# CederGroupHub/chgnet

Hardware: NVIDIA H100
Metric: structures_per_sec_EFS (higher is better)
Workload: dtype f32

## Files before the change

### chgnet_b200/_lib.py

```python
from __future__ import annotations

import ctypes
import os
from ctypes import c_char_p, c_double, c_float, c_int32, c_int64, c_void_p

import torch
from torch import Tensor

_HERE = os.path.dirname(os.path.abspath(__file__))
LIB_PATH = os.path.join(_HERE, "libchgnet_b200.so")

P, I, F, D, I64 = c_void_p, c_int32, c_float, c_double, c_int64

SIGNATURES: dict[str, list] = {
    "chg_embed_atoms": [P, P, I, P, P],
    "chg_edge_geometry": [P, P, P, P, P, P, I, P, P, P, P],
    "chg_bond_basis_embed": [P, P, I, P, P, I, F, F, I, P, P, P, P, P, P],
    "chg_bond_basis_bwd": [P, P, I, P, P, I, F, F, I, P, P, P, P, P, P, P],
    "chg_angle_basis_embed": [P, P, P, I, P, I, P, P, P, P],
    "chg_angle_basis_bwd": [P, P, P, I, P, I, P, P, P, P, P],
    "chg_linear": [P, P, I, I, P, P, P, P, I, P, P],
    "chg_gather_rows": [P, P, I, I, P, P],
    "chg_scatter_rows": [P, P, I, I, P, P],
    "chg_atom_conv_fwd": [P, P, P, P, P, P, I, P, P, P, P, P, P, P],
    "chg_atom_conv_bwd": [P, P, P, P, P, P, I, P, P, P, P, P, P, P, P, P],
    "chg_segment_sum": [P, I, P, P, I, I, I, P, I, P],
    "chg_atom_conv_fused": [P, P, P, P, P, P, P, I, I, P, P, P, P, P, P, P],
    "chg_bond_conv_fused": [P, P, P, P, P, P, P, P, I, I, P, P, P, P, P, P, P, P],
    "chg_bond_conv_fwd": [P, P, P, P, P, P, P, I, P, P, P, P, P, P, P],
    "chg_bond_conv_bwd": [P, P, P, P, P, I, P, P, P, P, P, P, P, P, P],
    "chg_angle_update_fwd": [P, P, P, P, P, P, P, I, P, P, P, P],
    "chg_angle_update_bwd": [P, P, I, P, P, P, P],
    "chg_readout": [P, P, P, I, P, P, P, P, I, P, F, P, P, P, P, P, P, P],
    "chg_magmom": [P, I, P, F, P, P],
    "chg_force_virial": [P, P, P, P, P, P, P, P, P, P, I, P, P, P],
    "chg_wgrad": [P, P, I, P, I, P, I, P, I, I, P, I, P, P, P],
    "chg_colsum": [P, I, P, I, P, I, I, P, P],
    "chg_readout_bwd": [P, I, P, P, P, P, I, P, P, P, P, P, P, P, P],
    "chg_magmom_bwd": [P, I, P, F, P, P, P, P],
    "chg_loss_terms": [P, P, I, I, F, P, P, P],
    "chg_adam_step": [P, P, P, P, I64, F, F, F, F, F, I, P],
    "chg_edge_tangent": [P, P, P, P, P, P, P, P, I, P, P, P],
    "chg_bond_basis_tangent": [P, P, P, I, P, P, I, F, F, I, P, P, P, P, P, P],
    "chg_bond_basis_bwd2": [P, P, P, I, P, P, I, F, F, I, P, P, P, P, P, P],
    "chg_angle_basis_tangent": [P, P, P, P, I, P, I, P, P, P, P],
    "chg_angle_basis_bwd2": [P, P, P, P, I, P, I, P, P, P, P],
    "chg_atom_conv_tan": [P, P, P, P, P, P, P, I, P, P, P, P, P, P, P, P],
    "chg_atom_conv_bwd2": [P, P, P, P, P, P, P, P, P, I, P, P, P, P, P, P, P, P, P],
    "chg_bond_conv_tan": [P, P, P, P, P, P, P, P, I, P, P, P, P, P, P, P, P],
    "chg_bond_conv_bwd2": [P, P, P, P, P, P, P, P, P, I, P, P, P, P, P, P, P, P, P, P],
    "chg_angle_update_tan": [P, P, P, P, P, P, P, I, P, P, P, P, P],
    "chg_angle_update_bwd2": [P, P, P, P, I, P, P, P, P],
    "chg_readout_bwd2": [P, P, I, P, P, P, P, I, P, P, P, P, P, P, P, P, P, P, P, P],
    "chg_bond_basis_hvp": [P, P, P, I, P, P, I, F, F, I, P, P, P, P, P, P],
    "chg_angle_basis_hvp": [P, P, P, P, I, P, I, P, P, P, P],
    "chg_edge_tangent_bwd": [P, P, P, P, P, P, P, P, P, P, I, P, P],
    "chg_edge_tangent_bwd_virial": [P, P, P, P, P, P, P, P, P, P, P, P, I, P, P, P],
    "chg_dynamical_matrices": [P, P, P, P, P, I, I, P, I, P, P],
    "chg_dynamical_matrix_derivatives": [P, P, P, P, P, I, I, P, I, P, P, P],
    "chg_tetrahedron_dos": [P, I, I, I, I, P, P, I, P, I, P, P, P, P, P],
    "chg_thermal_displacements": [P, P, I, I, P, I, D, P, P, P],
    "chg_joint_dos": [P, I, I, I, I, P, P, I, P, I, P, I, D, P, P, P],
    "chg_structure_factors": [P, P, P, P, P, P, P, P, I, I, I, D, P, P],
    "chg_broadened_spectrum": [P, P, I, I, I, I64, I, I64, P, I, D, P, I64, P, P],
    "chg_phonon_interaction": [P, P, P, P, P, P, I, I, I, I, I, P, P, I, P, I, D, P, I64, P, P],
    "chg_imag_self_energy": [P, I, I, I, I, P, I, P, P, I, P, P, I, D, P, I64, P, P],
    "chg_collision_rows": [P, I, I, I, I, P, I, P, P, I, P, P, I, D, P, I64, P, P],
    "chg_self_energy_spectrum": [P, I, I, I, I, P, I, P, I, P, I, P, P, I, D, P, I64, P, P],
}

DOS_MAX_CHUNKS = 512
TD_MAX_CHUNKS = 128
JDOS_MAX_CHUNKS = 64
SQW_MAX_CHUNKS = 64


def sqw_scratch_doubles(n_rows, n_modes, n_t, row0, group_size, n_freq):
    if n_rows <= 0:
        return 0
    groups = (row0 + n_rows - 1) // group_size - row0 // group_size + 1
    chunks = max(1, min(SQW_MAX_CHUNKS, -(-min(group_size, n_rows) * n_modes // 32)))
    return chunks * n_t * groups * n_freq


ISE_MAX_CHUNKS = 64


def ph3_scratch_doubles(n_q1, n_prim, n_super):
    return 4 * n_q1 * (n_prim * n_super + (3 * n_prim) ** 3)


def ise_scratch_doubles(n_q1, n_band, n_t):
    return 2 * n_q1 * n_band**3 + ISE_MAX_CHUNKS * n_t * n_band


def collision_scratch_doubles(n_q1, n_band):
    return 3 * n_q1 * n_band**3


SE_MAX_CHUNKS = 128


def se_scratch_doubles(n_band, n_freq, n_t):
    return SE_MAX_CHUNKS * n_t * n_band * n_freq

_lib = None


class ChgnetB200Error(RuntimeError):
    pass


def _mesh_args(name, mesh, freqs, tetrahedra, f64_names, f64_tensors):
    n1, n2, n3 = (int(n) for n in mesh)
# ... 104 lines not shown
                       g_freq=None):
        self._chk(dist, u2d, freq_ag, freq_bg, w3, g_e0, g_wag, g_wbg, g_dist, g_freq)
        self._call("chg_bond_basis_bwd", _p(dist), _p(u2d), u2d.shape[0], _p(freq_ag), _p(freq_bg),
                   freq_ag.shape[0], float(rc_ag), float(rc_bg), int(p), _p(w3), _p(g_e0), _p(g_wag), _p(g_wbg),
                   _p(g_dist), _p(g_freq))

    def angle_basis_embed(self, rhat, ang_di, ang_dj, freq, wt, a0, basis_out=None):
        self._chk(rhat, ang_di, ang_dj, freq, wt, a0, basis_out)
        self._call("chg_angle_basis_embed", _p(rhat), _p(ang_di), _p(ang_dj), ang_di.shape[0], _p(freq),
                   freq.shape[0], _p(wt), _p(a0), _p(basis_out))

    def angle_basis_bwd(self, rhat, ang_di, ang_dj, freq, w, g_a0, g_rhat, g_freq=None):
        self._chk(rhat, ang_di, ang_dj, freq, w, g_a0, g_rhat, g_freq)
        self._call("chg_angle_basis_bwd", _p(rhat), _p(ang_di), _p(ang_dj), ang_di.shape[0], _p(freq),
                   freq.shape[0], _p(w), _p(g_a0), _p(g_rhat), _p(g_freq))

    def linear(self, x, wt, bias, residual, y, x_rows=None, y_rows=None):
        self._chk(x, wt, bias, residual, y, x_rows, y_rows)
        m = x_rows.shape[0] if x_rows is not None else x.shape[0]
        self._call("chg_linear", _p(x), _p(x_rows), m, x.shape[1], _p(wt), _p(bias), _p(residual), _p(y_rows),
                   wt.shape[1], _p(y))

    def gather_rows(self, src, idx, dst):
        self._chk(src, idx, dst)
        self._call("chg_gather_rows", _p(src), _p(idx), idx.shape[0], src.shape[1], _p(dst))

    def scatter_rows(self, src, idx, dst):
        self._chk(src, idx, dst)
        self._call("chg_scatter_rows", _p(src), _p(idx), idx.shape[0], src.shape[1], _p(dst))

    def atom_conv_fwd(self, pcn, pe, wag, center, nbr, d2u, w2t, b2, ln, msg, save_p, save_pre=None):
        self._chk(pcn, pe, wag, center, nbr, d2u, w2t, b2, ln, msg, save_p, save_pre)
        self._call("chg_atom_conv_fwd", _p(pcn), _p(pe), _p(wag), _p(center), _p(nbr), _p(d2u), center.shape[0],
                   _p(w2t), _p(b2), _p(ln), _p(msg), _p(save_p), _p(save_pre))

    def atom_conv_bwd(self, pcn, pe, wag, center, nbr, d2u, save_p, g_agg, w2, ln, g_pre, g_w, g_p=None, g_ln=None):
        self._chk(pcn, pe, wag, center, nbr, d2u, save_p, g_agg, w2, ln, g_pre, g_w, g_p, g_ln)
        self._call("chg_atom_conv_bwd", _p(pcn), _p(pe), _p(wag), _p(center), _p(nbr), _p(d2u), center.shape[0],
                   _p(save_p), _p(g_agg), _p(w2), _p(ln), _p(g_pre), _p(g_w), _p(g_p), _p(g_ln))

    def _fused_work(self, n_rows: int, device) -> Tensor:
        need = int(self.lib.chg_gated_fused_workspace_floats(int(n_rows)))
        ws = getattr(self, "_fws", None)
        if ws is None or ws.device != device or ws.numel() < need:
            ws = torch.empty(need, dtype=torch.float32, device=device)
            self._fws = ws
        return ws

    def atom_conv_fused(self, pcn, pe, wag, center, nbr, d2u, ptr_c, w2t, b2, ln, agg, save_p):
        self._chk(pcn, pe, wag, center, nbr, d2u, ptr_c, w2t, b2, ln, agg, save_p)
        self._call("chg_atom_conv_fused", _p(pcn), _p(pe), _p(wag), _p(center), _p(nbr), _p(d2u), _p(ptr_c), center.shape[0],
                   agg.shape[0], _p(w2t), _p(b2), _p(ln), _p(agg), _p(save_p), _p(self._fused_work(center.shape[0], agg.device)))

    def bond_conv_fused(self, pij, px, pa, wbg, ang_atom, ang_i, ang_j, ptr_i, w2t, b2, ln, agg, save_pre, save_p):
        self._chk(pij, px, pa, wbg, ang_atom, ang_i, ang_j, ptr_i, w2t, b2, ln, agg, save_pre, save_p)
        self._call("chg_bond_conv_fused", _p(pij), _p(px), _p(pa), _p(wbg), _p(ang_atom), _p(ang_i), _p(ang_j), _p(ptr_i),
                   ang_i.shape[0], agg.shape[0], _p(w2t), _p(b2), _p(ln), _p(agg), _p(save_pre), _p(save_p),
                   _p(self._fused_work(ang_i.shape[0], agg.device)))

    def segment_sum(self, data, perm, ptr, accumulate, out):
        self._chk(data, perm, ptr)
        if not out.is_cuda or out.stride(1) != 1:
            raise ChgnetB200Error("segment_sum output must be a CUDA tensor with unit column stride")
        n_items = data.shape[0] if perm is None else perm.shape[0]
        self._call("chg_segment_sum", _p(data), data.shape[1], _p(perm), _p(ptr), ptr.shape[0] - 1, n_items,
                   int(accumulate), _p(out), out.stride(0))

    def bond_conv_fwd(self, pij, px, pa, wbg, ang_atom, ang_i, ang_j, w2t, b2, ln, upd, save_pre, save_p):
        self._chk(pij, px, pa, wbg, ang_atom, ang_i, ang_j, w2t, b2, ln, upd, save_pre, save_p)
        self._call("chg_bond_conv_fwd", _p(pij), _p(px), _p(pa), _p(wbg), _p(ang_atom), _p(ang_i), _p(ang_j),
                   ang_i.shape[0], _p(w2t), _p(b2), _p(ln), _p(upd), _p(save_pre), _p(save_p))

    def bond_conv_bwd(self, save_pre, save_p, wbg, ang_i, ang_j, g_agg, w2, ln, g_pre, gw_i, gw_j, g_p=None,
                      g_ln=None):
        self._chk(save_pre, save_p, wbg, ang_i, ang_j, g_agg, w2, ln, g_pre, gw_i, gw_j, g_p, g_ln)
        self._call("chg_bond_conv_bwd", _p(save_pre), _p(save_p), _p(wbg), _p(ang_i), _p(ang_j), ang_i.shape[0],
                   _p(g_agg), _p(w2), _p(ln), _p(g_pre), _p(gw_i), _p(gw_j), _p(g_p), _p(g_ln))

    def angle_update_fwd(self, pij, px, pa, ang, ang_atom, ang_i, ang_j, ln, ang_new, save_p):
        self._chk(pij, px, pa, ang, ang_atom, ang_i, ang_j, ln, ang_new, save_p)
        self._call("chg_angle_update_fwd", _p(pij), _p(px), _p(pa), _p(ang), _p(ang_atom), _p(ang_i), _p(ang_j),
                   ang_i.shape[0], _p(ln), _p(ang_new), _p(save_p))

    def angle_update_bwd(self, save_p, g_ang_in, ln, g_pre, g_ln=None):
        self._chk(save_p, g_ang_in, ln, g_pre, g_ln)
        self._call("chg_angle_update_bwd", _p(save_p), _p(g_ang_in), save_p.shape[0], _p(ln), _p(g_pre), _p(g_ln))

    @staticmethod
    def _chk_rows(*tensors: Tensor | None) -> None:
        for t in tensors:
            if t is not None and (not t.is_cuda or t.stride(-1) != 1):
                raise ChgnetB200Error("kernel arguments must be CUDA tensors with unit column stride")

    def _workspace(self, n_out: int, device) -> Tensor:
        ws = getattr(self, "_ws", None)
        if ws is None or ws.device != device:
            need = max(int(self.lib.chg_wgrad_workspace_floats(n)) for n in (64, 128, 256))
            ws = torch.empty(need, dtype=torch.float32, device=device)
            self._ws = ws
        return ws

    def wgrad(self, x, g, out, colsum=None, x_rows=None, g_rows=None, x_silu=False, x2=None):
        self._chk_rows(x, g, out, x2)
        self._chk(colsum, x_rows, g_rows)
        if x2 is not None and x2.stride(0) != x.stride(0):
            raise ChgnetB200Error("wgrad: x2 must have the row stride of x")
        m = x_rows.shape[0] if x_rows is not None else (g_rows.shape[0] if g_rows is not None else x.shape[0])
        self._call("chg_wgrad", _p(x), _p(x2), x.stride(0), _p(x_rows), int(bool(x_silu)), _p(g), g.stride(0), _p(g_rows), m,
                   out.shape[1], _p(out), out.stride(0), _p(colsum), _p(self._workspace(out.shape[1], x.device)))

    def colsum(self, a, out, b=None, rowscale=None):
        self._chk_rows(a, b)
        self._chk(out, rowscale)
        self._call("chg_colsum", _p(a), a.stride(0), _p(b), b.stride(0) if b is not None else 0, _p(rowscale),
                   a.shape[0], a.shape[1], _p(out))

    def readout_bwd(self, x, ln, mlp_wt, mlp_w, mlp_b, w_last, seed, g_x, h_all, gz_all, g_h0, xhat):
        self._chk(x, ln, mlp_wt, mlp_w, mlp_b, w_last, seed, g_x, h_all, gz_all, g_h0, xhat)
        self._call("chg_readout_bwd", _p(x), x.shape[0], _p(ln), _p(mlp_wt), _p(mlp_w), _p(mlp_b), mlp_wt.shape[0],
                   _p(w_last), _p(seed), _p(g_x), _p(h_all), _p(gz_all), _p(g_h0), _p(xhat))

    def magmom_bwd(self, x, w, b, g_m, g_x, g_lin):
        self._chk(x, w, g_m, g_x, g_lin)
        self._call("chg_magmom_bwd", _p(x), x.shape[0], _p(w), float(b), _p(g_m), _p(g_x), _p(g_lin))

    def loss_terms(self, pred, target, kind, delta, g_pred, sums):
        self._chk(pred, target, g_pred, sums)
        self._call("chg_loss_terms", _p(pred), _p(target), pred.numel(), int(kind), float(delta), _p(g_pred), _p(sums))

    def edge_tangent(self, rvec, dist, rhat, center, nbr, owner, u_atom, w_graph, ddist, drhat):
        self._chk(rvec, dist, rhat, center, nbr, owner, u_atom, w_graph, ddist, drhat)
        self._call("chg_edge_tangent", _p(rvec), _p(dist), _p(rhat), _p(center), _p(nbr), _p(owner), _p(u_atom),
                   _p(w_graph), center.shape[0], _p(ddist), _p(drhat))

    def bond_basis_tangent(self, dist, ddist, u2d, freq_ag, freq_bg, rc_ag, rc_bg, p, w3t, e0d, wagd, wbgd, tbasis):
        self._chk(dist, ddist, u2d, freq_ag, freq_bg, w3t, e0d, wagd, wbgd, tbasis)
        self._call("chg_bond_basis_tangent", _p(dist), _p(ddist), _p(u2d), u2d.shape[0], _p(freq_ag), _p(freq_bg),
                   freq_ag.shape[0], float(rc_ag), float(rc_bg), int(p), _p(w3t), _p(e0d), _p(wagd), _p(wbgd), _p(tbasis))

    def bond_basis_bwd2(self, dist, ddist, u2d, freq_ag, freq_bg, rc_ag, rc_bg, p, w3, lam_e0, lam_wag, lam_wbg, g_freq):
        self._chk(dist, ddist, u2d, freq_ag, freq_bg, w3, lam_e0, lam_wag, lam_wbg, g_freq)
        self._call("chg_bond_basis_bwd2", _p(dist), _p(ddist), _p(u2d), u2d.shape[0], _p(freq_ag), _p(freq_bg),
                   freq_ag.shape[0], float(rc_ag), float(rc_bg), int(p), _p(w3), _p(lam_e0), _p(lam_wag), _p(lam_wbg),
                   _p(g_freq))

    def angle_basis_tangent(self, rhat, drhat, ang_di, ang_dj, freq, wt, a0d, tbasis):
        self._chk(rhat, drhat, ang_di, ang_dj, freq, wt, a0d, tbasis)
        self._call("chg_angle_basis_tangent", _p(rhat), _p(drhat), _p(ang_di), _p(ang_dj), ang_di.shape[0], _p(freq),
                   freq.shape[0], _p(wt), _p(a0d), _p(tbasis))

    def angle_basis_bwd2(self, rhat, drhat, ang_di, ang_dj, freq, w, lam_a0, g_freq):
        self._chk(rhat, drhat, ang_di, ang_dj, freq, w, lam_a0, g_freq)
        self._call("chg_angle_basis_bwd2", _p(rhat), _p(drhat), _p(ang_di), _p(ang_dj), ang_di.shape[0], _p(freq),
                   freq.shape[0], _p(w), _p(lam_a0), _p(g_freq))

    def bond_basis_hvp(self, dist, ddist, u2d, freq_ag, freq_bg, rc_ag, rc_bg, p, w3, lam_e0, lam_wag, lam_wbg, g_dist):
        self._chk(dist, ddist, u2d, freq_ag, freq_bg, w3, lam_e0, lam_wag, lam_wbg, g_dist)
        self._call("chg_bond_basis_hvp", _p(dist), _p(ddist), _p(u2d), u2d.shape[0], _p(freq_ag), _p(freq_bg),
                   freq_ag.shape[0], float(rc_ag), float(rc_bg), int(p), _p(w3), _p(lam_e0), _p(lam_wag), _p(lam_wbg),
                   _p(g_dist))

    def angle_basis_hvp(self, rhat, drhat, ang_di, ang_dj, freq, w, lam_a0, g_rhat):
        self._chk(rhat, drhat, ang_di, ang_dj, freq, w, lam_a0, g_rhat)
        self._call("chg_angle_basis_hvp", _p(rhat), _p(drhat), _p(ang_di), _p(ang_dj), ang_di.shape[0], _p(freq),
                   freq.shape[0], _p(w), _p(lam_a0), _p(g_rhat))

# ... 251 lines not shown
```

### chgnet_b200/csrc/native_engine.cu

```cuda
#include <cstdarg>
#include <cstdio>
#include <cstring>
#include <string>

#include "common.cuh"

namespace chg {
namespace {

constexpr size_t ALIGN = 256;
constexpr int64_t PAD = 16;

struct GatedW {
  const float *w2t = nullptr, *w2 = nullptr, *b2 = nullptr, *ln = nullptr;
  const float *a_t = nullptr, *b_t = nullptr, *c_t = nullptr, *bias1 = nullptr;
  const float *a_b = nullptr, *b_b = nullptr, *c_b = nullptr;
  const float *wo_t = nullptr, *wo = nullptr, *bo = nullptr;
};
struct Weights {
  const float *emb, *freq_ag, *freq_bg, *freq_ang, *w3t, *w3, *wang_t, *wang;
  GatedW atom[CHG_MAX_CONV], bond[CHG_MAX_CONV], angle[CHG_MAX_CONV];
  const float *readout_ln, *mlp_wt, *mlp_w, *mlp_b, *w_last, *w_mag, *atom_ref;
};

// ... 147 lines not shown
      rc = CHG_ERR_CUDA;
    }
  }
};

#define RUN(c, name, call) \
  do {                     \
    if ((c).go(name)) (c).rc = (call); \
  } while (0)

int run_schedule(const chg_hparams& hp, const Weights& W, const chg_batch& b, const chg_outputs& o, Ctx& c) {
  const int N = b.n_atoms, Ed = b.n_edges, Eu = b.n_bonds, A = b.n_angles, B = b.n_graphs, Es = b.n_short;
  const bool has_ang = A > 0;
  const bool grad = o.force != nullptr || o.virial != nullptr;
  const int n_conv = hp.n_conv;
  void* st = c.stream;
  auto lin = [&](const float* x, const int32_t* xr, int m, int k, const float* wt, const float* bias, const float* res,
                 const int32_t* yr, int n, float* y) { RUN(c, "linear", chg_linear(x, xr, m, k, wt, bias, res, yr, n, y, st)); };
  auto seg = [&](const float* data, int width, const int32_t* perm, const int32_t* ptr, int rows, int items, int acc,
                 float* out, int ld) { RUN(c, "segment_sum", chg_segment_sum(data, width, perm, ptr, rows, items, acc, out, ld, st)); };

  float* x = c.f(true, (size_t)N * 64);
  RUN(c, "embed_atoms", chg_embed_atoms(b.z, W.emb, N, x, st));
  float *rvec = c.f(true, (size_t)Ed * 3), *dist = c.f(true, Ed), *rhat = c.f(true, (size_t)Ed * 3);
  RUN(c, "edge_geometry", chg_edge_geometry(b.frac, b.lattice, b.owner, b.center, b.nbr, b.image, Ed, rvec, dist, rhat, st));
  float *e = c.f(true, (size_t)Eu * 64), *wag = c.f(true, (size_t)Eu * 64), *wbg = c.f(true, (size_t)Eu * 64);
  RUN(c, "bond_basis_embed", chg_bond_basis_embed(dist, b.u2d, Eu, W.freq_ag, W.freq_bg, hp.num_radial, hp.atom_graph_cutoff,
                                                  hp.bond_graph_cutoff, hp.cutoff_coeff, W.w3t, e, wag, wbg, nullptr, st));
  float *ang = nullptr, *ang_alt = nullptr, *wbg_s = nullptr;
  if (has_ang) {
    ang = c.f(true, (size_t)A * 64);
    ang_alt = c.f(true, (size_t)A * 64);
    RUN(c, "angle_basis_embed", chg_angle_basis_embed(rhat, b.ang_di, b.ang_dj, A, W.freq_ang, (hp.num_angular - 1) / 2,
                                                      W.wang_t, ang, nullptr, st));
    wbg_s = c.f(true, (size_t)Es * 64);
    RUN(c, "gather_rows", chg_gather_rows(wbg, b.short_ids, Es, 64, wbg_s, st));
  }
  struct SavedAtom { float *pcn, *pe, *p; } sa[CHG_MAX_CONV];
  struct SavedBond { float *pre, *p; } sb[CHG_MAX_CONV];
  float* sang[CHG_MAX_CONV];

  auto atom_conv = [&](int t, const float* xin, float* xout) {
    const GatedW& g = W.atom[t];
    float* pcn = c.f(grad, (size_t)N * 256);
    float* pe = c.f(grad, (size_t)Eu * 128);
    lin(xin, nullptr, N, 64, g.a_t, nullptr, nullptr, nullptr, 256, pcn);
    lin(e, nullptr, Eu, 64, g.b_t, g.bias1, nullptr, nullptr, 128, pe);
    float* save_p = grad ? c.f(true, (size_t)Ed * 128) : nullptr;
    float* agg = c.f(false, (size_t)N * 64);
    float* work = c.f(false, (size_t)chg_gated_fused_workspace_floats(Ed));
    RUN(c, "atom_conv_fused", chg_atom_conv_fused(pcn, pe, wag, b.center, b.nbr, b.d2u, b.ptr_c, Ed, N, g.w2t, g.b2, g.ln, agg, save_p,
                                                  work, st));
    sa[t] = SavedAtom{pcn, pe, save_p};
    lin(agg, nullptr, N, 64, g.wo_t, g.bo, xin, nullptr, 64, xout);
    c.ar.reset_tmp();
  };

  float* x_mag = nullptr;
  for (int t = 0; t < n_conv - 1; ++t) {
    float* xn = (t == n_conv - 2 && o.atom_fea != nullptr) ? o.atom_fea : c.f(true, (size_t)N * 64);
    atom_conv(t, x, xn);
    x = xn;
    if (has_ang) {
      const GatedW& g = W.bond[t];
      float* pij = c.f(false, (size_t)Es * 256);
      float* px = c.f(false, (size_t)N * 128);
      float* pa = c.f(false, (size_t)A * 128);
      lin(e, b.short_ids, Es, 64, g.a_t, g.bias1, nullptr, nullptr, 256, pij);
      lin(x, nullptr, N, 64, g.b_t, nullptr, nullptr, nullptr, 128, px);
      lin(ang, nullptr, A, 64, g.c_t, nullptr, nullptr, nullptr, 128, pa);
      float* s_pre = grad ? c.f(true, (size_t)A * 128) : nullptr;
      float* s_p = grad ? c.f(true, (size_t)A * 128) : nullptr;
      float* agg = c.f(false, (size_t)Es * 64);
      float* work = c.f(false, (size_t)chg_gated_fused_workspace_floats(A));
      RUN(c, "bond_conv_fused", chg_bond_conv_fused(pij, px, pa, wbg_s, b.ang_atom, b.ang_is, b.ang_js, b.ptr_is, A, Es, g.w2t, g.b2,
                                                    g.ln, agg, s_pre, s_p, work, st));
      lin(agg, nullptr, Es, 64, g.wo_t, g.bo, e, b.short_ids, 64, e);
      sb[t] = SavedBond{s_pre, s_p};
      c.ar.reset_tmp();
      if (t < n_conv - 2) {
        const GatedW& ga = W.angle[t];
        pij = c.f(false, (size_t)Es * 256);
        px = c.f(false, (size_t)N * 128);
        pa = c.f(false, (size_t)A * 128);
        lin(e, b.short_ids, Es, 64, ga.a_t, ga.bias1, nullptr, nullptr, 256, pij);
        lin(x, nullptr, N, 64, ga.b_t, nullptr, nullptr, nullptr, 128, px);
        lin(ang, nullptr, A, 64, ga.c_t, nullptr, nullptr, nullptr, 128, pa);
        float* s_pa = grad ? c.f(true, (size_t)A * 128) : nullptr;
        RUN(c, "angle_update_fwd", chg_angle_update_fwd(pij, px, pa, ang, b.ang_atom, b.ang_is, b.ang_js, A, ga.ln, ang_alt, s_pa, st));
        sang[t] = s_pa;
        float* sw = ang;
        ang = ang_alt;
        ang_alt = sw;
        c.ar.reset_tmp();
      }
    }
    if (t == n_conv - 2) {
      x_mag = x;
      if (o.magmom != nullptr) RUN(c, "magmom", chg_magmom(x, N, W.w_mag, hp.b_mag, o.magmom, st));
    }
  }
  if (n_conv == 1 && o.magmom != nullptr) c.zero(o.magmom, (size_t)N * 4);
  (void)x_mag;
  {
    float* xn = c.f(true, (size_t)N * 64);
    atom_conv(n_conv - 1, x, xn);
    x = xn;
  }

  float* h_out = o.crystal_fea != nullptr ? c.f(false, (size_t)N * 64) : nullptr;
  float* g_x = grad ? c.f(true, (size_t)N * 64) : nullptr;
  c.zero(o.energy, (size_t)B * 8);
  c.zero(o.e_ref, (size_t)B * 8);
  RUN(c, "readout", chg_readout(x, b.z, b.owner, N, W.readout_ln, W.mlp_wt, W.mlp_w, W.mlp_b, hp.n_readout_hidden, W.w_last,
                                hp.b_last, W.atom_ref, o.site_e, h_out, o.energy, o.e_ref, g_x, st));
  if (o.crystal_fea != nullptr) seg(h_out, 64, nullptr, b.graph_ptr, B, N, 0, o.crystal_fea, 64);
  c.ar.reset_tmp();
  if (!grad) return c.rc;

  float* g_e = c.f(true, (size_t)Eu * 64);
  bool g_e_live = false;
  float* g_wag = c.f(true, (size_t)Eu * 64);
  c.zero(g_wag, (size_t)Eu * 256);
  float* g_wbg = has_ang ? c.f(true, (size_t)Es * 64) : nullptr;
  if (has_ang) c.zero(g_wbg, (size_t)Es * 256);
  float* g_a = has_ang ? c.f(true, (size_t)A * 64) : nullptr;
  bool g_a_live = false;

  auto atom_bwd = [&](int t) {
    const GatedW& g = W.atom[t];
    float* g_agg = c.f(false, (size_t)N * 64);
    lin(g_x, nullptr, N, 64, g.wo, nullptr, nullptr, nullptr, 64, g_agg);
    float* g_pre = c.f(false, (size_t)Ed * 128);
    float* g_w = c.f(false, (size_t)Ed * 64);
    RUN(c, "atom_conv_bwd", chg_atom_conv_bwd(sa[t].pcn, sa[t].pe, wag, b.center, b.nbr, b.d2u, Ed, sa[t].p, g_agg, g.w2, g.ln,
                                              g_pre, g_w, nullptr, nullptr, st));
    float* sp = c.f(false, (size_t)N * 256);
    seg(g_pre, 128, nullptr, b.ptr_c, N, Ed, 0, sp, 256);
    seg(g_pre, 128, b.perm_n, b.ptr_n, N, Ed, 0, sp + 128, 256);
    lin(sp, nullptr, N, 256, g.a_b, nullptr, g_x, nullptr, 64, g_x);
    float* spe = c.f(false, (size_t)Eu * 128);
    seg(g_pre, 128, b.perm_u, b.ptr_u, Eu, Ed, 0, spe, 128);
    lin(spe, nullptr, Eu, 128, g.b_b, nullptr, g_e_live ? g_e : nullptr, nullptr, 64, g_e);
    g_e_live = true;
    seg(g_w, 64, b.perm_u, b.ptr_u, Eu, Ed, 1, g_wag, 64);
    c.ar.reset_tmp();
  };
  auto angle_scatter = [&](const float* g_pre, const GatedW& g) {
    float* sp = c.f(false, (size_t)Es * 256);
    seg(g_pre, 128, nullptr, b.ptr_is, Es, A, 0, sp, 256);
    seg(g_pre, 128, b.perm_js, b.ptr_js, Es, A, 0, sp + 128, 256);
    lin(sp, nullptr, Es, 256, g.a_b, nullptr, g_e, b.short_ids, 64, g_e);
    float* spx = c.f(false, (size_t)N * 128);
    seg(g_pre, 128, b.perm_x, b.ptr_x, N, A, 0, spx, 128);
    lin(spx, nullptr, N, 128, g.b_b, nullptr, g_x, nullptr, 64, g_x);
  };

  atom_bwd(n_conv - 1);
  for (int t = n_conv - 2; t >= 0; --t) {
    if (has_ang) {
      if (t < n_conv - 2) {
        const GatedW& ga = W.angle[t];
        float* g_pre = c.f(false, (size_t)A * 128);
        RUN(c, "angle_update_bwd", chg_angle_update_bwd(sang[t], g_a_live ? g_a : nullptr, A, ga.ln, g_pre, nullptr, st));
        lin(g_pre, nullptr, A, 128, ga.c_b, nullptr, g_a_live ? g_a : nullptr, nullptr, 64, g_a);
        g_a_live = true;
        angle_scatter(g_pre, ga);
        c.ar.reset_tmp();
      }
      const GatedW& g = W.bond[t];
      float* g_agg = c.f(false, (size_t)Es * 64);
      lin(g_e, b.short_ids, Es, 64, g.wo, nullptr, nullptr, nullptr, 64, g_agg);
// ... 174 lines not shown
```

### chgnet_b200/engine.py

```python
from __future__ import annotations

from dataclasses import dataclass, field

import torch
from torch import Tensor

from chgnet_b200.batch import DeviceBatch
from chgnet_b200.weights import PackedWeights

EV_A3_TO_GPA = 160.21766208


@dataclass
class EngineOutput:
    energy: Tensor
    e_ref: Tensor
    site_e: Tensor
    magmom: Tensor | None = None
    atom_fea: Tensor | None = None
    crystal_fea: Tensor | None = None
    force: Tensor | None = None
    virial: Tensor | None = None
    extras: dict = field(default_factory=dict)

# ... 45 lines not shown
        K.embed_atoms(b.z, pw.emb, x)
        rvec, dist, rhat = self._new(b, Ed, 3), self._new(b, Ed), self._new(b, Ed, 3)
        K.edge_geometry(b.frac, b.lattice, b.owner, b.center, b.nbr, b.image, rvec, dist, rhat)
        e, wag, wbg = self._new(b, Eu, 64), self._new(b, Eu, 64), self._new(b, Eu, 64)
        tr: dict = dict(x=[], e=[], ang=[], agg_a=[], agg_b=[]) if train else {}
        if train:
            tr["bb"] = self._new(b, Eu, 64)
            K.bond_basis_embed(dist, b.u2d, pw.freq_ag, pw.freq_bg, hp.atom_graph_cutoff, hp.bond_graph_cutoff,
                               hp.cutoff_coeff, pw.w3t, e, wag, wbg, tr["bb"])
        else:
            K.bond_basis_embed(dist, b.u2d, pw.freq_ag, pw.freq_bg, hp.atom_graph_cutoff, hp.bond_graph_cutoff,
                               hp.cutoff_coeff, pw.w3t, e, wag, wbg)
        ang = None
        if has_ang:
            ang = self._new(b, A, 64)
            if train:
                tr["fb"] = self._new(b, A, 64)
                K.angle_basis_embed(rhat, b.ang_di, b.ang_dj, pw.freq_ang, pw.wang_t, ang, tr["fb"])
            else:
                K.angle_basis_embed(rhat, b.ang_di, b.ang_dj, pw.freq_ang, pw.wang_t, ang)
        if keep_intermediates:
            inter.update(x0=x, e0=e, w_ag=wag, w_bg=wbg, a0=ang)

        saved_atom: list[dict] = []
        saved_bond: list[dict] = []
        saved_angle: list[dict] = []

        def atom_conv(t: int, x: Tensor, e: Tensor) -> Tensor:
            gp = pw.atom[t]
            pcn = self._lin(b, x, gp.extra["wcn_t"])
            pe = self._lin(b, e, gp.extra["we_t"], bias=gp.extra["b1"])
            save_p = self._new(b, Ed, 128) if need_grad else None
            agg = self._new(b, N, 64)
            if train:
                msg = self._new(b, Ed, 64)
                save_pre = self._new(b, Ed, 128)
                K.atom_conv_fwd(pcn, pe, wag, b.center, b.nbr, b.d2u, gp.w2t, gp.b2, gp.ln, msg, save_p, save_pre)
                K.segment_sum(msg, None, b.ptr_c, 0, agg)
            else:
                K.atom_conv_fused(pcn, pe, wag, b.center, b.nbr, b.d2u, b.ptr_c, gp.w2t, gp.b2, gp.ln, agg, save_p)
            if need_grad:
                saved_atom.append(dict(pcn=pcn, pe=pe, p=save_p))
            if train:
                saved_atom[-1].update(pre=save_pre, x=x, e=e, agg=agg)
            return self._lin(b, agg, gp.extra["wo_t"], bias=gp.extra["bo"], residual=x)

        Es, sid = b.n_short, b.short_ids
        wbg_s = None
        if has_ang:
            wbg_s = self._new(b, Es, 64)
            K.gather_rows(wbg, sid, wbg_s)

        magmom = atom_fea = None
        for t in range(n_conv - 1):
            x = atom_conv(t, x, e)
            if has_ang:
                gp = pw.bond[t]
                pij = self._lin(b, e, gp.extra["wij_t"], bias=gp.extra["bij"], x_rows=sid)
                px = self._lin(b, x, gp.extra["wx_t"])
                pa = self._lin(b, ang, gp.extra["w1a_t"])
                s_pre = self._new(b, A, 128) if need_grad else None
                s_p = self._new(b, A, 128) if need_grad else None
                agg = self._new(b, Es, 64)
                if train:
                    upd = self._new(b, A, 64)
                    K.bond_conv_fwd(pij, px, pa, wbg_s, b.ang_atom, b.ang_is, b.ang_js, gp.w2t, gp.b2, gp.ln,
                                    upd, s_pre, s_p)
                    K.segment_sum(upd, None, b.ptr_is, 0, agg)
                else:
                    K.bond_conv_fused(pij, px, pa, wbg_s, b.ang_atom, b.ang_is, b.ang_js, b.ptr_is, gp.w2t, gp.b2, gp.ln,
                                      agg, s_pre, s_p)
                e_in = e
                if keep_intermediates or train:
                    e = e.clone()
                K.linear(agg, gp.extra["wo_t"], gp.extra["bo"], e, e, None, sid)
                if need_grad:
                    saved_bond.append(dict(pre=s_pre, p=s_p))
                if train:
                    saved_bond[-1].update(x=x, e=e_in, ang=ang, agg=agg)
                if t < n_conv - 2:
                    ga = pw.angle[t]
                    pij = self._lin(b, e, ga.extra["wij_t"], bias=ga.extra["bij"], x_rows=sid)
                    px = self._lin(b, x, ga.extra["wx_t"])
                    pa = self._lin(b, ang, ga.extra["w1a_t"])
                    ang_new = self._new(b, A, 64)
                    s_p = self._new(b, A, 128) if need_grad else None
                    K.angle_update_fwd(pij, px, pa, ang, b.ang_atom, b.ang_is, b.ang_js, ga.ln, ang_new, s_p)
                    if need_grad:
                        saved_angle.append(dict(p=s_p))
                    if train:
                        saved_angle[-1].update(x=x, e=e, ang=ang)
                    ang = ang_new
            if keep_intermediates:
                inter[f"x{t + 1}"], inter[f"e{t + 1}"] = x, e
                if t < n_conv - 2:
                    inter[f"a{t + 1}"] = ang
            if t == n_conv - 2:
                if need_atom_fea:
                    atom_fea = x
                if need_magmom:
                    magmom = self._new(b, N)
                    K.magmom(x, pw.w_mag, pw.b_mag, magmom)
                    tr["x_mag"] = x
        x = atom_conv(n_conv - 1, x, e)

        site_e = self._new(b, N)
        h_out = self._new(b, N, 64) if (need_crystal_fea or keep_intermediates) else None
        energy = self._zeros(b, B, dtype=torch.float64)
        e_ref = self._zeros(b, B, dtype=torch.float64)
        g_x = self._new(b, N, 64) if need_grad else None
        K.readout(x, b.z, b.owner, pw.readout_ln, pw.mlp_wt, pw.mlp_w, pw.mlp_b, pw.w_last, pw.b_last,
                  pw.atom_ref, site_e, h_out, energy, e_ref, g_x)
        crystal_fea = None
        if need_crystal_fea:
            gptr = torch.zeros(B + 1, dtype=torch.int32, device=b.z.device)
            gptr[1:] = torch.cumsum(torch.tensor(b.atoms_per_graph, device=b.z.device), 0)
            crystal_fea = self._seg(b, h_out, None, gptr, B)
        if keep_intermediates:
            inter["x_readout"], inter["site_e_model"] = h_out, site_e
        out = EngineOutput(energy=energy, e_ref=e_ref, site_e=site_e, magmom=magmom, atom_fea=atom_fea,
                           crystal_fea=crystal_fea, extras=inter)
        if not need_grad:
            return out
        st = dict(b=b, x_last=x, g_x=g_x, wag=wag, wbg_s=wbg_s, dist=dist, rvec=rvec, rhat=rhat, tr=tr,
                  saved_atom=saved_atom, saved_bond=saved_bond, saved_angle=saved_angle)
        if train:
            out.extras["train_state"] = st
            return out
        self._reverse(st, out, None)
        return out

    def input_grads(self, out: EngineOutput, record: bool = False) -> None:
        st = out.extras["train_state"]
        n = self.pw.hp.n_conv
        rec = dict(atom=[None] * n, bond=[None] * (n - 1), angle=[None] * (n - 1)) if record else None
        self._reverse(st, out, None, rec)
        if record:
            st["rec"] = rec

    def param_grads(self, out: EngineOutput, seed_energy: Tensor, seed_magmom: Tensor | None = None,
                    seed_force: Tensor | None = None, seed_stress: Tensor | None = None) -> dict:
        st = out.extras.pop("train_state")
        grads: dict = {}
        if seed_force is not None or seed_stress is not None:
            if "rec" not in st:
                raise RuntimeError("call input_grads(out, record=True) before param_grads with force / stress seeds")
            self._second_order(st, dict(seed_energy=seed_energy, seed_magmom=seed_magmom, seed_force=seed_force,
                                        seed_stress=seed_stress, grads=grads))
            return grads
        self._reverse(st, out, dict(seed_energy=seed_energy, seed_magmom=seed_magmom, grads=grads))
        return grads

    def hessian_vector_products(self, b: DeviceBatch, directions: Tensor) -> Tensor:
        out = self.run(b, need_grad=True, train=True)
        self.input_grads(out, record=True)
        st = out.extras.pop("train_state")
        return self._second_order(st, dict(seed_energy=self._zeros(b, b.n_graphs, dtype=torch.float64), seed_magmom=None,
                                           seed_force=None, seed_stress=None, grads=None, directions=directions))[0]

    def second_derivatives(self, b: DeviceBatch, directions: Tensor, strain_directions: Tensor) -> tuple[Tensor, Tensor]:
        out = self.run(b, need_grad=True, train=True)
        self.input_grads(out, record=True)
        st = out.extras.pop("train_state")
        hv, dt_dstrain = self._second_order(st, dict(
            seed_energy=self._zeros(b, b.n_graphs, dtype=torch.float64), seed_magmom=None, seed_force=None,
            seed_stress=None, grads=None, directions=directions, strain_directions=strain_directions))
        return hv, dt_dstrain.view(b.n_graphs, 3, 3)

    def _second_order(self, st: dict, train: dict) -> tuple[Tensor, Tensor] | None:
        pw, K, hp = self.pw, self.K, self.pw.hp
# ... 436 lines not shown
```

### include/chgnet_b200.h

```cpp
#ifndef CHGNET_B200_H
#define CHGNET_B200_H

#include <stdint.h>

#ifdef __cplusplus
extern "C" {
#endif

#define CHG_FEA 64
#define CHG_MAX_CONV 8
#define CHG_MAX_Z 94
#define CHG_OK 0
#define CHG_ERR_ARG (-1)
#define CHG_ERR_CUDA (-2)

const char* chg_last_error(void);
int chg_abi_version(void);
int64_t chg_launch_count(void);
int chg_set_option(const char* name, int32_t value);

int chg_embed_atoms(const int32_t* z, const float* emb, int32_t n_atoms, float* x, void* stream);

int chg_edge_geometry(const float* frac, const float* lattice, const int32_t* atom_owner,
                      const int32_t* center, const int32_t* nbr, const float* image,
                      int32_t n_edges, float* rvec, float* dist, float* rhat, void* stream);

int chg_bond_basis_embed(const float* dist, const int32_t* u2d, int32_t n_bonds,
                         const float* freq_ag, const float* freq_bg, int32_t n_radial,
                         float rc_ag, float rc_bg, int32_t p, const float* w3t,
                         float* e0, float* wag, float* wbg,
                         float* basis_out ,
                         void* stream);
int chg_bond_basis_bwd(const float* dist, const int32_t* u2d, int32_t n_bonds,
                       const float* freq_ag, const float* freq_bg, int32_t n_radial,
                       float rc_ag, float rc_bg, int32_t p, const float* w3,
                       const float* g_e0, const float* g_wag, const float* g_wbg,
                       float* g_dist,
                       double* g_freq ,
                       void* stream);

int chg_angle_basis_embed(const float* rhat, const int32_t* ang_di, const int32_t* ang_dj,
                          int32_t n_angles, const float* freq, int32_t n_freq,
                          const float* wt, float* a0,
                          float* basis_out ,
                          void* stream);
int chg_angle_basis_bwd(const float* rhat, const int32_t* ang_di, const int32_t* ang_dj,
                        int32_t n_angles, const float* freq, int32_t n_freq,
                        const float* w, const float* g_a0, double* g_rhat ,
                        double* g_freq , void* stream);

int chg_linear(const float* x, const int32_t* x_rows, int32_t m, int32_t k, const float* wt,
               const float* bias, const float* residual, const int32_t* y_rows, int32_t n_out,
               float* y, void* stream);
int chg_gather_rows(const float* src, const int32_t* idx, int32_t n, int32_t width, float* dst,
                    void* stream);
int chg_scatter_rows(const float* src, const int32_t* idx, int32_t n, int32_t width, float* dst,
                     void* stream);

int chg_atom_conv_fwd(const float* pcn, const float* pe, const float* wag,
                      const int32_t* center, const int32_t* nbr, const int32_t* d2u,
                      int32_t n_edges, const float* w2t, const float* b2, const float* ln,
                      float* msg, float* save_p, float* save_pre ,
                      void* stream);
int chg_atom_conv_bwd(const float* pcn, const float* pe, const float* wag,
                      const int32_t* center, const int32_t* nbr, const int32_t* d2u,
                      int32_t n_edges, const float* save_p, const float* g_agg,
                      const float* w2, const float* ln, float* g_pre, float* g_w,
                      float* g_p ,
                      double* g_ln , void* stream);

int chg_segment_sum(const float* data, int32_t width, const int32_t* perm,
                    const int32_t* ptr, int32_t n_rows,
                    int32_t n_items , int32_t accumulate,
                    float* out, int32_t out_ld , void* stream);

int64_t chg_gated_fused_workspace_floats(int32_t n_rows);
int chg_atom_conv_fused(const float* pcn, const float* pe, const float* wag, const int32_t* center,
                        const int32_t* nbr, const int32_t* d2u, const int32_t* ptr_c, int32_t n_edges,
                        int32_t n_atoms, const float* w2t, const float* b2, const float* ln, float* agg,
                        float* save_p, float* work, void* stream);
int chg_bond_conv_fused(const float* pij, const float* px, const float* pa, const float* wbg,
                        const int32_t* ang_atom, const int32_t* ang_i, const int32_t* ang_j,
                        const int32_t* ptr_i, int32_t n_angles, int32_t n_slots, const float* w2t,
                        const float* b2, const float* ln, float* agg, float* save_pre, float* save_p,
                        float* work, void* stream);

int chg_bond_conv_fwd(const float* pij, const float* px, const float* pa, const float* wbg,
                      const int32_t* ang_atom, const int32_t* ang_i, const int32_t* ang_j,
                      int32_t n_angles, const float* w2t, const float* b2, const float* ln,
                      float* upd, float* save_pre, float* save_p, void* stream);
int chg_bond_conv_bwd(const float* save_pre, const float* save_p, const float* wbg,
                      const int32_t* ang_i, const int32_t* ang_j, int32_t n_angles,
                      const float* g_agg, const float* w2, const float* ln, float* g_pre,
                      float* gw_i, float* gw_j, float* g_p ,
                      double* g_ln , void* stream);

int chg_angle_update_fwd(const float* pij, const float* px, const float* pa, const float* ang,
                         const int32_t* ang_atom, const int32_t* ang_i, const int32_t* ang_j,
                         int32_t n_angles, const float* ln, float* ang_new, float* save_p,
                         void* stream);
int chg_angle_update_bwd(const float* save_p, const float* g_ang_in, int32_t n_angles,
                         const float* ln, float* g_pre, double* g_ln ,
                         void* stream);

int chg_readout(const float* x, const int32_t* z, const int32_t* atom_owner, int32_t n_atoms,
                const float* ln, const float* mlp_wt, const float* mlp_w, const float* mlp_b,
                int32_t n_hidden, const float* w_last, float b_last, const float* atom_ref,
                float* site_e, float* h_out, double* e_graph, double* e_ref, float* g_x,
                void* stream);
int chg_magmom(const float* x, int32_t n_atoms, const float* w, float b, float* m, void* stream);

int chg_force_virial(const float* rvec, const float* dist, const float* rhat,
                     const double* g_rhat, const float* g_dist, const int32_t* d2u,
                     const int32_t* u2d, const int32_t* center, const int32_t* nbr,
                     const int32_t* atom_owner, int32_t n_edges, double* force,
                     double* virial, void* stream);

typedef struct {
  int32_t num_radial;
  int32_t num_angular;
  int32_t n_conv;
  int32_t cutoff_coeff;
  int32_t n_readout_hidden;
  int32_t use_ln;
  int32_t readout_ln;
  int32_t has_mlp_out_bias;
  float atom_graph_cutoff;
  float bond_graph_cutoff;
  float b_last;
  float b_mag;
} chg_hparams;

typedef struct {
  const float* core_w1; const float* core_b1; const float* gate_w1; const float* gate_b1;
  const float* core_w2; const float* core_b2; const float* gate_w2; const float* gate_b2;
  const float* ln1_w; const float* ln1_b; const float* ln2_w; const float* ln2_b;
  const float* out_w; const float* out_b;
} chg_gated_sd;
typedef struct {
  const float* atom_embedding;
  const float* freq_ag; const float* freq_bg; const float* freq_ang;
  const float* bond_embedding; const float* bond_weights_ag; const float* bond_weights_bg;
  const float* angle_embedding;
  chg_gated_sd atom[CHG_MAX_CONV];
  chg_gated_sd bond[CHG_MAX_CONV];
  chg_gated_sd angle[CHG_MAX_CONV];
  const float* readout_ln_w; const float* readout_ln_b;
  const float* mlp_w[4]; const float* mlp_b[4];
  const float* mlp_last_w; float mlp_last_b;
  const float* site_wise_w; float site_wise_b;
  const float* atom_ref;
} chg_state_dict;
int64_t chg_packed_floats(const chg_hparams* hp);
int chg_pack_weights_host(chg_hparams* hp, const chg_state_dict* sd, float* packed_host);

typedef struct {
  int32_t n_atoms, n_edges, n_bonds, n_angles, n_graphs, n_short;
  const int32_t* z; const float* frac; const int32_t* owner; const float* lattice;
  const int32_t* center; const int32_t* nbr; const float* image;
  const int32_t* d2u; const int32_t* u2d;
  const int32_t* ptr_c; const int32_t* perm_n; const int32_t* ptr_n; const int32_t* perm_u; const int32_t* ptr_u;
  const int32_t* ang_atom; const int32_t* ang_di; const int32_t* ang_dj; const int32_t* ang_is; const int32_t* ang_js;
  const int32_t* ptr_is; const int32_t* perm_js; const int32_t* ptr_js; const int32_t* perm_x; const int32_t* ptr_x;
  const int32_t* short_ids;
  const int32_t* graph_ptr;
} chg_batch;
typedef struct {
  double* energy; double* e_ref; float* site_e;
  float* magmom; float* atom_fea; float* crystal_fea;
  double* force; double* virial;
} chg_outputs;
int chg_forward_plan(const chg_hparams* hp, const chg_batch* sizes, const chg_outputs* wanted,
                     size_t* workspace_bytes, char* trace, size_t trace_cap);
int chg_forward(const chg_hparams* hp, const float* packed_weights, const chg_batch* batch,
                const chg_outputs* out, void* workspace , size_t workspace_bytes,
                void* stream);

typedef struct chg_graph chg_graph;
int chg_graph_build(const double* frac, const double* lattice, int32_t n_atoms, double r_atom, double r_bond,
                    chg_graph** out);
void chg_graph_sizes(const chg_graph* g, int64_t* n_edges, int64_t* n_bonds, int64_t* n_angles);
int chg_graph_export(const chg_graph* g, int32_t* atom_graph, float* image, int32_t* d2u, int32_t* u2d,
                     int32_t* bond_graph);
// ... 180 lines not shown
```

Measured before the change: 10920.

## Fuse angle-update linear projection into tensor-core WGMMA angle update kernel

Adds a new persistent kernel that computes the angle-feature projection (ang @ Wc) with 3xTF32 WGMMA on H100 and fuses the gather-add of pij/px, layer norm, gating and residual into the same kernel. The native engine and the inference path in the Python engine use it instead of a separate linear launch followed by the old update kernel. This removes the A x 128 intermediate buffer write and read plus one launch per angle layer. The trade-off is extra split-precision MMA work and per-block weight staging in shared memory; the training path keeps the old kernel.

```diff
diff --git a/chgnet_b200/_lib.py b/chgnet_b200/_lib.py
--- a/chgnet_b200/_lib.py
+++ b/chgnet_b200/_lib.py
@@ -30,6 +30,7 @@
     "chg_bond_conv_fwd": [P, P, P, P, P, P, P, I, P, P, P, P, P, P, P],
     "chg_bond_conv_bwd": [P, P, P, P, P, I, P, P, P, P, P, P, P, P, P],
     "chg_angle_update_fwd": [P, P, P, P, P, P, P, I, P, P, P, P],
+    "chg_angle_update_fwd_tc": [P, P, P, P, P, P, P, I, P, P, P, P],
     "chg_angle_update_bwd": [P, P, I, P, P, P, P],
     "chg_readout": [P, P, P, I, P, P, P, P, I, P, F, P, P, P, P, P, P, P],
     "chg_magmom": [P, I, P, F, P, P],
@@ -300,6 +301,11 @@
         self._call("chg_angle_update_fwd", _p(pij), _p(px), _p(pa), _p(ang), _p(ang_atom), _p(ang_i), _p(ang_j),
                    ang_i.shape[0], _p(ln), _p(ang_new), _p(save_p))
 
+    def angle_update_fwd_tc(self, pij, px, ang, wc, ang_atom, ang_i, ang_j, ln, ang_new, save_p):
+        self._chk(pij, px, ang, wc, ang_atom, ang_i, ang_j, ln, ang_new, save_p)
+        self._call("chg_angle_update_fwd_tc", _p(pij), _p(px), _p(ang), _p(wc), _p(ang_atom), _p(ang_i), _p(ang_j),
+                   ang_i.shape[0], _p(ln), _p(ang_new), _p(save_p))
+
     def angle_update_bwd(self, save_p, g_ang_in, ln, g_pre, g_ln=None):
         self._chk(save_p, g_ang_in, ln, g_pre, g_ln)
         self._call("chg_angle_update_bwd", _p(save_p), _p(g_ang_in), save_p.shape[0], _p(ln), _p(g_pre), _p(g_ln))
diff --git a/chgnet_b200/csrc/angle_ws.cu b/chgnet_b200/csrc/angle_ws.cu
--- /dev/null
+++ b/chgnet_b200/csrc/angle_ws.cu
@@ -0,0 +1,235 @@
+#include "gated_common.cuh"
+#include "tc.cuh"
+
+namespace chg {
+namespace gated {
+namespace {
+
+constexpr int AT_THREADS = 256;
+constexpr int AT_TR = 128;
+constexpr int AT_IMG_BYTES = 128 * 64 * 4;
+
+struct AngleSmem {
+  static constexpr int IMG_OFF = 0;
+  static constexpr int ANG_OFF = 2 * AT_IMG_BYTES;
+  static constexpr int IDX_OFF = ANG_OFF + AT_TR * 64 * 4;
+  static constexpr int LN_OFF = IDX_OFF + 3 * AT_TR * 4;
+  static constexpr int TOTAL = LN_OFF + 256 * 4;
+};
+
+struct AngleArgs {
+  const float* pij;
+  const float* px;
+  const float* ang;
+  const float* wc;
+  const int32_t* ang_atom;
+  const int32_t* ang_i;
+  const int32_t* ang_j;
+  int32_t n_rows;
+  const float* ln;
+  float* ang_new;
+  float* save_p;
+};
+
+__device__ __forceinline__ int swz(int r, int c) { return r * 256 + ((c ^ (r & 7)) << 4); }
+__device__ __forceinline__ void prefetch_l2(const void* p) { asm volatile("prefetch.global.L2 [%0];" ::"l"(p)); }
+
+__device__ __forceinline__ float quad_tree_sum(const float (&x)[16]) {
+  float s[8];
+#pragma unroll
+  for (int j = 0; j < 8; ++j) {
+    const float y0 = __shfl_xor_sync(0xffffffffu, x[2 * j], 1), y1 = __shfl_xor_sync(0xffffffffu, x[2 * j + 1], 1);
+    const float p = ((x[2 * j] + x[2 * j + 1]) + y0) + y1;
+    s[j] = p + __shfl_xor_sync(0xffffffffu, p, 2);
+  }
+  const float t = ((s[0] + s[1]) + (s[2] + s[3])) + ((s[4] + s[5]) + (s[6] + s[7]));
+  return __shfl_sync(0xffffffffu, t, (threadIdx.x & 31) & ~3);
+}
+
+__device__ __forceinline__ void ln_frag(float (&d)[64], int blk, int h, const float* s_gamma, const float* s_beta) {
+  float x[16];
+#pragma unroll
+  for (int j = 0; j < 8; ++j) {
+    x[2 * j] = d[blk * 32 + 4 * j + 2 * h];
+    x[2 * j + 1] = d[blk * 32 + 4 * j + 2 * h + 1];
+  }
+  const float mean = quad_tree_sum(x) * (1.f / 64.f);
+  float sq[16];
+#pragma unroll
+  for (int j = 0; j < 8; ++j) {
+    const float e0 = x[2 * j] - mean, e1 = x[2 * j + 1] - mean;
+    const float f0 = __shfl_xor_sync(0xffffffffu, e0, 1), f1 = __shfl_xor_sync(0xffffffffu, e1, 1);
+    sq[2 * j] = fmaf(f1, f1, fmaf(f0, f0, fmaf(e1, e1, fmaf(e0, e0, 0.f))));
+    sq[2 * j + 1] = 0.f;
+  }
+  float s[8];
+#pragma unroll
+  for (int j = 0; j < 8; ++j) s[j] = sq[2 * j] + __shfl_xor_sync(0xffffffffu, sq[2 * j], 2);
+  const float var = __shfl_sync(0xffffffffu, ((s[0] + s[1]) + (s[2] + s[3])) + ((s[4] + s[5]) + (s[6] + s[7])),
+                                (threadIdx.x & 31) & ~3) * (1.f / 64.f);
+  const float rstd = 1.f / sqrtf(var + LN_EPS);
+#pragma unroll
+  for (int j = 0; j < 8; ++j) {
+#pragma unroll
+    for (int e = 0; e < 2; ++e) {
+      const int i = blk * 32 + 4 * j + 2 * h + e;
+      const int c = tc::frag_col(i) - blk * 64;
+      d[i] = fmaf((d[i] - mean) * rstd, s_gamma[c], s_beta[c]);
+    }
+  }
+}
+
+__device__ __forceinline__ void wg_gemm_ang(float (&d)[64], const uint8_t* s_ang, int row0, uint32_t bhi, uint32_t blo) {
+  const int lane = threadIdx.x & 31;
+  int r = row0 + 16 * ((threadIdx.x >> 5) & 3) + (lane >> 2);
+  asm volatile("mov.b32 %0, %0;" : "+r"(r));
+  const int c = lane & 3;
+  auto at = [&](int rr, int k) { return *reinterpret_cast<const float*>(s_ang + swz(rr, k >> 2) + (k & 3) * 4); };
+#pragma unroll
+  for (int q = 0; q < 4; ++q) {
+    uint32_t ahi[2][4], alo[2][4];
+#pragma unroll
+    for (int j = 0; j < 2; ++j) {
+      const int k = (q * 2 + j) * 8 + c;
+      tc::split_tf32(at(r, k), ahi[j][0], alo[j][0]);
+      tc::split_tf32(at(r + 8, k), ahi[j][1], alo[j][1]);
+      tc::split_tf32(at(r, k + 4), ahi[j][2], alo[j][2]);
+      tc::split_tf32(at(r + 8, k + 4), ahi[j][3], alo[j][3]);
+    }
+    tc::wgmma_fence();
+#pragma unroll
+    for (int j = 0; j < 2; ++j) {
+      const uint32_t koff = (uint32_t)(q * 2 + j) * 256;
+      const uint64_t bh = tc::smem_desc_kmajor(bhi + koff, 128, 2048), bl = tc::smem_desc_kmajor(blo + koff, 128, 2048);
+      tc::wgmma_tf32_m64n128(d, ahi[j], bh);
+      tc::wgmma_tf32_m64n128(d, alo[j], bh);
+      tc::wgmma_tf32_m64n128(d, ahi[j], bl);
+    }
+    tc::wgmma_commit();
+    tc::wgmma_wait<0>();
+  }
+}
+
+__global__ void __launch_bounds__(AT_THREADS, 2) angle_tc_fwd_kernel(const AngleArgs a) {
+  extern __shared__ __align__(1024) uint8_t smem_raw[];
+  uint8_t* s_img = smem_raw + AngleSmem::IMG_OFF;
+  uint8_t* s_ang = smem_raw + AngleSmem::ANG_OFF;
+  int* s_idx = reinterpret_cast<int*>(smem_raw + AngleSmem::IDX_OFF);
+  float* s_ln = reinterpret_cast<float*>(smem_raw + AngleSmem::LN_OFF);
+
+  const int tid = threadIdx.x;
+  const bool use_ln = a.ln != nullptr;
+  const int n_tiles = (a.n_rows + AT_TR - 1) / AT_TR;
+
+  for (int i = tid; i < 128 * 64; i += AT_THREADS) {
+    const int kk = i >> 7, n = i & 127;
+    uint32_t h, l;
+    tc::split_tf32(__ldg(a.wc + i), h, l);
+    const uint32_t off = tc::kmajor_offset(n, kk, 64);
+    *reinterpret_cast<uint32_t*>(s_img + off) = h;
+    *reinterpret_cast<uint32_t*>(s_img + AT_IMG_BYTES + off) = l;
+  }
+  s_ln[tid] = use_ln ? a.ln[tid] : 0.f;
+  tc::fence_async_smem();
+
+  const int row0 = (tid >> 7) * 64;
+  const uint32_t img = tc::smem_u32(s_img);
+  for (int tile = blockIdx.x; tile < n_tiles; tile += gridDim.x) {
+    const int base = tile * AT_TR;
+    __syncthreads();
+    if (tid < AT_TR) {
+      const int r = min(base + tid, a.n_rows - 1);
+      s_idx[tid] = a.ang_i[r];
+      s_idx[AT_TR + tid] = a.ang_j[r];
+      s_idx[2 * AT_TR + tid] = a.ang_atom[r];
+    }
+    {
+      float4 v[8];
+#pragma unroll
+      for (int p = 0; p < 8; ++p) {
+        const int r = min(base + p * 16 + (tid >> 4), a.n_rows - 1);
+        v[p] = ldg4(a.ang + (size_t)r * 64 + (tid & 15) * 4);
+      }
+#pragma unroll
+      for (int p = 0; p < 8; ++p) *reinterpret_cast<float4*>(s_ang + swz(p * 16 + (tid >> 4), tid & 15)) = v[p];
+      const int nt = tile + gridDim.x;
+      if (nt < n_tiles) prefetch_l2(a.ang + (size_t)min(nt * AT_TR + (tid & 127), a.n_rows - 1) * 64 + (tid >> 7) * 32);
+    }
+    __syncthreads();
+
+    float d[64];
+#pragma unroll
+    for (int i = 0; i < 64; ++i) d[i] = 0.f;
+    wg_gemm_ang(d, s_ang, row0, img, img + AT_IMG_BYTES);
+
+    const int lr = row0 + tc::frag_row(0);
+#pragma unroll
+    for (int h = 0; h < 2; ++h) {
+      const float* s0 = a.pij + (size_t)s_idx[lr + 8 * h] * 256;
+      const float* s1 = a.pij + (size_t)s_idx[AT_TR + lr + 8 * h] * 256 + 128;
+      const float* s2 = a.px + (size_t)s_idx[2 * AT_TR + lr + 8 * h] * 128;
+#pragma unroll
+      for (int i = 2 * h; i < 64; i += 4) {
+        const int c = tc::frag_col(i);
+        const float2 v0 = __ldg(reinterpret_cast<const float2*>(s0 + c));
+        const float2 v1 = __ldg(reinterpret_cast<const float2*>(s1 + c));
+        const float2 v2 = __ldg(reinterpret_cast<const float2*>(s2 + c));
+        d[i] = (v0.x + v1.x + v2.x) + d[i];
+        d[i + 1] = (v0.y + v1.y + v2.y) + d[i + 1];
+      }
+    }
+    if (a.save_p != nullptr) {
+#pragma unroll
+      for (int i = 0; i < 64; i += 2) {
+        const int g = base + row0 + tc::frag_row(i);
+        if (g < a.n_rows) *reinterpret_cast<float2*>(a.save_p + (size_t)g * 128 + tc::frag_col(i)) = make_float2(d[i], d[i + 1]);
+      }
+    }
+    if (use_ln) {
+#pragma unroll
+      for (int h = 0; h < 2; ++h) {
+        ln_frag(d, 0, h, s_ln, s_ln + 64);
+        ln_frag(d, 1, h, s_ln + 128, s_ln + 192);
+      }
+    }
+#pragma unroll
+    for (int i = 0; i < 32; i += 2) {
+      const int r = row0 + tc::frag_row(i), c = tc::frag_col(i), g = base + r;
+      const float2 res = *reinterpret_cast<const float2*>(s_ang + swz(r, c >> 2) + (c & 3) * 4);
+      const float2 o = make_float2(silu_f(d[i]) * sigmoid_f(d[i + 32]) + res.x, silu_f(d[i + 1]) * sigmoid_f(d[i + 33]) + res.y);
+      if (g < a.n_rows) *reinterpret_cast<float2*>(a.ang_new + (size_t)g * 64 + c) = o;
+    }
+  }
+}
+
+int launch_angle_tc_fwd(const AngleArgs& a, cudaStream_t stream) {
+  static int slots_of[MAX_DEVICES] = {};
+  int& slots = slots_of[device_ordinal()];
+  if (slots == 0) {
+    CHG_CUDA(cudaFuncSetAttribute(angle_tc_fwd_kernel, cudaFuncAttributeMaxDynamicSharedMemorySize, AngleSmem::TOTAL));
+    int per_sm = 0;
+    if (cudaOccupancyMaxActiveBlocksPerMultiprocessor(&per_sm, angle_tc_fwd_kernel, AT_THREADS, AngleSmem::TOTAL) != cudaSuccess ||
+        per_sm < 1)
+      per_sm = 1;
+    slots = per_sm * sm_count();
+  }
+  const int n_tiles = (a.n_rows + AT_TR - 1) / AT_TR;
+  angle_tc_fwd_kernel<<<min(n_tiles, slots), AT_THREADS, AngleSmem::TOTAL, stream>>>(a);
+  CHG_LAUNCH_END();
+}
+
+}
+}
+}
+
+using namespace chg;
+
+extern "C" int chg_angle_update_fwd_tc(const float* pij, const float* px, const float* ang, const float* wc,
+                                       const int32_t* ang_atom, const int32_t* ang_i, const int32_t* ang_j,
+                                       int32_t n_angles, const float* ln, float* ang_new, float* save_p, void* stream) {
+  CHG_CHECK_ARG(n_angles >= 0, "negative size");
+  if (n_angles == 0) return CHG_OK;
+  CHG_CHECK_ARG(pij && px && ang && wc && ang_atom && ang_i && ang_j && ang_new, "null pointer");
+  gated::AngleArgs a{pij, px, ang, wc, ang_atom, ang_i, ang_j, n_angles, ln, ang_new, save_p};
+  return gated::launch_angle_tc_fwd(a, as_stream(stream));
+}
diff --git a/chgnet_b200/csrc/native_engine.cu b/chgnet_b200/csrc/native_engine.cu
--- a/chgnet_b200/csrc/native_engine.cu
+++ b/chgnet_b200/csrc/native_engine.cu
@@ -253,12 +253,11 @@
         const GatedW& ga = W.angle[t];
         pij = c.f(false, (size_t)Es * 256);
         px = c.f(false, (size_t)N * 128);
-        pa = c.f(false, (size_t)A * 128);
         lin(e, b.short_ids, Es, 64, ga.a_t, ga.bias1, nullptr, nullptr, 256, pij);
         lin(x, nullptr, N, 64, ga.b_t, nullptr, nullptr, nullptr, 128, px);
-        lin(ang, nullptr, A, 64, ga.c_t, nullptr, nullptr, nullptr, 128, pa);
         float* s_pa = grad ? c.f(true, (size_t)A * 128) : nullptr;
-        RUN(c, "angle_update_fwd", chg_angle_update_fwd(pij, px, pa, ang, b.ang_atom, b.ang_is, b.ang_js, A, ga.ln, ang_alt, s_pa, st));
+        RUN(c, "angle_update_fwd",
+            chg_angle_update_fwd_tc(pij, px, ang, ga.c_t, b.ang_atom, b.ang_is, b.ang_js, A, ga.ln, ang_alt, s_pa, st));
         sang[t] = s_pa;
         float* sw = ang;
         ang = ang_alt;
diff --git a/chgnet_b200/engine.py b/chgnet_b200/engine.py
--- a/chgnet_b200/engine.py
+++ b/chgnet_b200/engine.py
@@ -151,10 +151,17 @@
                     ga = pw.angle[t]
                     pij = self._lin(b, e, ga.extra["wij_t"], bias=ga.extra["bij"], x_rows=sid)
                     px = self._lin(b, x, ga.extra["wx_t"])
-                    pa = self._lin(b, ang, ga.extra["w1a_t"])
                     ang_new = self._new(b, A, 64)
                     s_p = self._new(b, A, 128) if need_grad else None
-                    K.angle_update_fwd(pij, px, pa, ang, b.ang_atom, b.ang_is, b.ang_js, ga.ln, ang_new, s_p)
+                    fwd_tc = None if train else getattr(K, "angle_update_fwd_tc", None)
+                    if train:
+                        pa = self._lin(b, ang, ga.extra["w1a_t"])
+                        K.angle_update_fwd(pij, px, pa, ang, b.ang_atom, b.ang_is, b.ang_js, ga.ln, ang_new, s_p)
+                    elif fwd_tc is not None:
+                        fwd_tc(pij, px, ang, ga.extra["w1a_t"], b.ang_atom, b.ang_is, b.ang_js, ga.ln, ang_new, s_p)
+                    else:
+                        K.angle_update_fwd(pij, px, ang @ ga.extra["w1a_t"], ang, b.ang_atom, b.ang_is, b.ang_js,
+                                           ga.ln, ang_new, s_p)
                     if need_grad:
                         saved_angle.append(dict(p=s_p))
                     if train:
diff --git a/include/chgnet_b200.h b/include/chgnet_b200.h
--- a/include/chgnet_b200.h
+++ b/include/chgnet_b200.h
@@ -99,6 +99,10 @@
                          const int32_t* ang_atom, const int32_t* ang_i, const int32_t* ang_j,
                          int32_t n_angles, const float* ln, float* ang_new, float* save_p,
                          void* stream);
+int chg_angle_update_fwd_tc(const float* pij, const float* px, const float* ang, const float* wc,
+                            const int32_t* ang_atom, const int32_t* ang_i, const int32_t* ang_j,
+                            int32_t n_angles, const float* ln, float* ang_new, float* save_p,
+                            void* stream);
 int chg_angle_update_bwd(const float* save_p, const float* g_ang_in, int32_t n_angles,
                          const float* ln, float* g_pre, double* g_ln ,
                          void* stream);
```

Measured after the change: 11120 (median of 6 runs). +1.8%, better.
